# lucadellalib/audiocodecs

Hardware: AMD Instinct MI355X
Metric: encode+decode audio-sec/s, EnCodec-24k 8cb (higher is better)
Workload: dtype f32 (GEMM-shaped kernels and LSTM products: operands as two scaled fp16 planes, 3 partial products, fp32 accumulate -- split16.h)

## Files before the change

### audiocodecs_amd/csrc/ac_api.hip

```cpp
#include "core.h"
#include "tap_route.h"

extern "C" {

int ac_version(void) { return 400; }

int ac_create(const ac_config* cfg, ac_handle** out) {
    if (!cfg || !out) return AC_EINVAL;
    *out = nullptr;
    if (cfg->struct_size != (int32_t)sizeof(ac_config)) return AC_EINVAL;
    if (cfg->num_ratios < 1 || cfg->num_ratios > AC_MAX_RATIOS || cfg->num_filters < 1 || cfg->hidden_size < 16 ||
        cfg->hidden_size % 16 || cfg->compress < 1 || cfg->num_lstm_layers < 1 || cfg->num_lstm_layers > 2 || cfg->codebook_size % 32 ||
        cfg->codebook_size < 16 || cfg->num_quantizers < 1 || cfg->kernel_size < 1 || cfg->kernel_size > 8 ||
        cfg->last_kernel_size < 1 || cfg->last_kernel_size > 8 || cfg->residual_kernel_size < 1 || cfg->residual_kernel_size > 8)
        return AC_EINVAL;
    int ndev = 0;
    if (hipGetDeviceCount(&ndev) != hipSuccess || ndev <= cfg->device || cfg->device < 0) return AC_ENODEV;
    ac_handle* h = new (std::nothrow) ac_handle();
    if (!h) return AC_ENOMEM;
    h->cfg = *cfg;
    h->hop = 1;
    for (int i = 0; i < cfg->num_ratios; ++i) h->hop *= cfg->upsampling_ratios[i];
    h->D = cfg->num_filters << cfg->num_ratios;
    *out = h;
// ... 9 lines not shown
static std::string wavtok_key(const std::string& name) {
    static const std::string pre = "feature_extractor.encodec.encoder.model.";
    if (name.compare(0, pre.size(), pre) != 0) return name;
    std::string k = "encoder.layers." + name.substr(pre.size());
    const size_t cc = k.find(".conv.conv.");
    if (cc != std::string::npos) k = k.substr(0, cc) + ".conv." + k.substr(cc + 11);
    auto ends = [&](const char* sfx) { const size_t n = std::strlen(sfx); return k.size() >= n && k.compare(k.size() - n, n, sfx) == 0; };
    if (ends(".weight_g")) k = k.substr(0, k.size() - 9) + ".parametrizations.weight.original0";
    else if (ends(".weight_v")) k = k.substr(0, k.size() - 9) + ".parametrizations.weight.original1";
    return k;
}

int ac_load_weights(ac_handle* h, const char* name, const void* host_ptr, size_t bytes) {
    if (!h || !name || !host_ptr) return h ? fail(h, AC_EINVAL, "null argument") : AC_EINVAL;
    if (h->finalized) return fail(h, AC_ESTATE, "handle already finalized");
    if (bytes % 4) return fail(h, AC_EINVAL, "tensor '%s': byte size %zu is not a multiple of 4", name, bytes);
    const float* f = static_cast<const float*>(host_ptr);
    h->host[h->arch == ARCH_WAVTOK ? wavtok_key(name) : std::string(name)].assign(f, f + bytes / 4);
    return AC_OK;
}



static void latch_dev_switches(ac_handle* h) {
    auto num = [](const char* name, int dflt) { const char* v = std::getenv(name); return v && *v ? std::atoi(v) : dflt; };
    const char* e = std::getenv("AC_TAP_EPI");
    h->dev.tap_epi_staged = e && std::strcmp(e, "staged") == 0;
    h->dev.tap_dil = num("AC_TAP_DIL", 1);
    h->dev.tap_stagger = num("AC_TAP_STAGGER", 0);
    h->dev.tap_pick = num("AC_TAP_PICK", -1);
    h->dev.tap8 = num("AC_TAP8", -1);
    h->dev.tap8_form = num("AC_TAP8_FORM", 0);
    h->dev.tap8_spread = num("AC_TAP8_SPREAD", 1);
#ifdef AC_DEVELOPER
    h->dev.rb6_dbg = num("AC_RB6_DBG", 0);
    h->dev.lstm_dbg = num("AC_LSTM_DBG", 0);
#endif
    h->dev.rb_stream = num("AC_RB_STREAM", 1);
    h->dev.chain_stream = num("AC_CHAIN_STREAM", 1);
    h->dev.rb128_stream = num("AC_RB128_STREAM", 1);
    h->dev.front_seg = std::max(0, num("AC_FRONT_SEG", 0));
    h->dev.tail_seg = std::max(0, num("AC_TAIL_SEG", 0));
    h->dev.front_ldspad = std::max(0, num("AC_FRONT_LDSPAD", 0));
    h->dev.lstm_fuse_in = num("AC_LSTM_FUSE_IN", 1);
    const char* r = std::getenv("AC_RVQ");
    h->dev.rvq_exact = r && std::strcmp(r, "fp32") == 0;
    h->dev.prof_detail = num("AC_PROF_DETAIL", 0);
    h->dev.head_seq = num("AC_HEAD_SEQ", 0);
    h->dev.attn_exact = num("AC_ATTN_EXACT", 0);
    h->dev.dac_unit = num("AC_DAC_UNIT", 1);
    h->dev.mimi_tail = num("AC_MIMI_TAIL", 1);
    h->dev.mstream_skinny = num("AC_MSTREAM_SKINNY", -1);
}

int ac_debug_set(ac_handle* h, const char* key, int value) {
    if (!h || !key) return AC_EINVAL;
    struct { const char* k; int* v; } tab[] = {
        {"tap_epi_staged", &h->dev.tap_epi_staged}, {"tap_dil", &h->dev.tap_dil}, {"tap_stagger", &h->dev.tap_stagger}, {"tap_pick", &h->dev.tap_pick}, {"tap8", &h->dev.tap8}, {"tap8_form", &h->dev.tap8_form}, {"tap8_spread", &h->dev.tap8_spread},
        {"rb6_dbg", &h->dev.rb6_dbg}, {"rb_stream", &h->dev.rb_stream}, {"chain_stream", &h->dev.chain_stream}, {"rb128_stream", &h->dev.rb128_stream}, {"front_seg", &h->dev.front_seg}, {"tail_seg", &h->dev.tail_seg}, {"front_ldspad", &h->dev.front_ldspad},
        {"lstm_dbg", &h->dev.lstm_dbg}, {"lstm_fuse_in", &h->dev.lstm_fuse_in}, {"rvq_exact", &h->dev.rvq_exact}, {"prof_detail", &h->dev.prof_detail}, {"head_seq", &h->dev.head_seq}, {"attn_exact", &h->dev.attn_exact}, {"dac_unit", &h->dev.dac_unit}, {"mimi_tail", &h->dev.mimi_tail},
        {"mstream_skinny", &h->dev.mstream_skinny},
    };
#ifndef AC_DEVELOPER
    if (std::strcmp(key, "rb6_dbg") == 0 || std::strcmp(key, "lstm_dbg") == 0)
        return fail(h, AC_EINVAL, "ac_debug_set('%s'): a developer-build switch (timing modes with wrong results / fault injection); this is the product library", key);
#endif
    if (!h->finalized) return fail(h, AC_ESTATE, "ac_debug_set('%s'): the switches are latched by ac_finalize; set them afterwards", key);
    for (auto& t : tab)
        if (std::strcmp(t.k, key) == 0) {
            const bool nonneg = t.v == &h->dev.front_seg || t.v == &h->dev.tail_seg || t.v == &h->dev.front_ldspad || t.v == &h->dev.tap_stagger;
            if (nonneg && value < 0) return fail(h, AC_EINVAL, "ac_debug_set('%s', %d): the value must be >= 0", key, value);
            if (t.v == &h->dev.front_ldspad && value > 16384) return fail(h, AC_EINVAL, "ac_debug_set('front_ldspad', %d): at most 16384 bytes", value);
            if (t.v == &h->dev.tap8_form && (value < 0 || value > 5)) return fail(h, AC_EINVAL, "ac_debug_set('tap8_form', %d): 0 (cost model) .. 5", value);
            *t.v = value;
            return AC_OK;
        }
    return fail(h, AC_EINVAL, "ac_debug_set: unknown switch '%s'", key);
}

int ac_set_precision(ac_handle* h, int precision) {
    if (!h) return AC_EINVAL;
    if (h->finalized) return fail(h, AC_ESTATE, "ac_set_precision must precede ac_finalize (weights are packed for one arithmetic)");
    if (precision != AC_PRECISION_FP32 && precision != AC_PRECISION_FP32_EXACT) return fail(h, AC_EINVAL, "unknown precision %d", precision);
    h->precision = precision;
    return AC_OK;
}

int ac_finalize(ac_handle* h) {
    if (!h) return AC_EINVAL;
    if (h->finalized) return fail(h, AC_ESTATE, "handle already finalized");
    {
// ... 552 lines not shown
```

### audiocodecs_amd/csrc/core.h

```cpp
#pragma once
#include <hip/hip_runtime.h>

#include <algorithm>
#include <cmath>
#include <cstdarg>
#include <cstdio>
#include <cstdlib>
#include <cstring>
#include <map>
#include <string>
#include <vector>

#include "../../include/audiocodecs_amd.h"
#include "lstm_consts.h"
#include "rvq_types.h"
#include "split16.h"
#include "tap_gemm.h"

using namespace ac;

namespace ac {
constexpr int THIN_MAXK = 8;
struct RbFused6Params;
}
// ... 113 lines not shown
    int arch = ARCH_ENCODEC;
    ac_config cfg{};
    ac_mimi_config mcfg{};
    MimiPlan mimi;
    ac_dac_config dcfg{};
    DacPlan dac;
    ac_wavtok_config wcfg{};
    WavtokPlan wt;
    std::string err;
    std::map<std::string, std::vector<float>> host;
    bool finalized = false;
    float* blob = nullptr;
    size_t blob_floats = 0;
    int hop = 1, D = 0;
    PackedGemm enc_stem, enc_final;
    std::vector<ResBlockPlan> enc_rb;
    std::vector<PackedGemm> enc_down;
    LstmPlan enc_lstm, dec_lstm;
    PackedGemm dec_first, dec_head;
    std::vector<PackedGemm> dec_up;
    std::vector<ResBlockPlan> dec_rb;
    size_t cb_plain = 0, cb_packed = 0, cb_ee = 0;
    size_t cb16 = 0, cb16_inv = 0;
    struct ChainBounds { float sb0 = 0.f, sb1 = 0.f, fb0 = 0.f, fb1h = 0.f, fb1x = 0.f; bool ok = false; } enc_front, dec_tail;
    struct StreamImgs { size_t stem_f = 0, stem_inv = 0, down_f = 0, down_inv = 0, up_f = 0, up_inv = 0, head_f = 0, head_inv = 0; bool enc_ok = false, dec_ok = false; } simg;
    struct DevSwitches {
        int tap_epi_staged = 0;
        int tap_dil = 1;
        int tap_stagger = 0;
        int tap_pick = -1;
        int tap8 = -1;
        int tap8_form = 0;
        int tap8_spread = 1;
        int rb6_dbg = 0;
        int rb_stream = 1;
        int rb128_stream = 1;
        int chain_stream = 1;
        int front_seg = 0, tail_seg = 0;
        int front_ldspad = 0;
        int lstm_dbg = 0;
        int lstm_fuse_in = 1;
        int rvq_exact = 0;
        int prof_detail = 0;
        int attn_exact = 0;
        int dac_unit = 1;
        int mimi_tail = 1;
        int head_seq = 0;
        int mstream_skinny = -1;
    } dev;
    bool fuse_chains = true;
    float* dbg = nullptr;
    size_t dbg_cap = 0, dbg_used = 0;
    std::vector<const void*> lds_opted;
    std::map<size_t, size_t> w6_of;
    std::map<size_t, size_t> t6_of;
    std::map<size_t, size_t> t6inv_of;
    bool noncausal = false;
    bool has_enc = true, has_dec = true;
    bool gemm_fp32 = false;
    std::map<size_t, size_t> winv_of;
    std::map<const void*, int> mimi_streams;
    std::map<const void*, int> mimi_dstreams;
    struct EStreamReg { int B; bool fresh; };
    std::map<const void*, EStreamReg> encodec_streams, encodec_dstreams;
    unsigned* amax_buf = nullptr;
    int amax_B = 0, amax_next = 0;
// ... 744 lines not shown
```

### audiocodecs_amd/csrc/core.hip

```cpp
#include "core.h"
#include "split16_kernels.h"
#include "lstm.h"
#include "lstm_persist.h"
#include "lstm_persist16.h"
#include "rvq.h"
#include "rvq16.h"
#include "tap_gemm4.h"
#include "tap_gemm6.h"
#include "tap_gemm8.h"
#include "tap_route.h"
#include "thin.h"
#include "rb_fused.h"
#include "rb_fused6.h"
#include "thin_conv6.h"
#include "rb_fused6_128.h"
#include "enc_front.h"
#include "dec_tail.h"

namespace acimpl {


int fail(ac_handle* h, int code, const char* fmt, ...) {
    char buf[1024];
    va_list ap;
// ... 176 lines not shown
static int launch_tap6(ac_handle* h, hipStream_t st, TapGemmParams& p, const __bf16* w6, const char* name, double flops, double bytes) {
    using Cfg = Tap6Cfg<WGM, WGN, WMT, WN, HALO>;
    p.mtiles = cdiv(p.M, Cfg::BM);
    p.ntiles = p.N / Cfg::BN;
    const long long blocks = (long long)p.B * p.mtiles * p.ntiles;
    if (int rc = ensure_lds(h, reinterpret_cast<const void*>(tap_gemm6_kernel<WGM, WGN, WMT, WN, 2, HALO>), Cfg::lds_for(2))) return rc;
    ProfScope ps(h, st, name, flops, bytes);
    hipLaunchKernelGGL((tap_gemm6_kernel<WGM, WGN, WMT, WN, 2, HALO>), dim3((unsigned)blocks), dim3(Cfg::NT), Cfg::lds_for(2), st, p, w6);
    return AC_OK;
}

static int launch_tap6_family(ac_handle* h, hipStream_t st, TapGemmParams& p, const TapRoute& r, const __bf16* w6, const char* name, double flops, double bytes) {
    if (r.family == TapFamily::tap6_dil) {
        switch (r.key()) {
        case tap_key(1, 4, 4, 2): return launch_tap6<1, 4, 4, 2, T6_DIL_HALO>(h, st, p, w6, name, flops, bytes);
        case tap_key(1, 4, 4, 1): return launch_tap6<1, 4, 4, 1, T6_DIL_HALO>(h, st, p, w6, name, flops, bytes);
        case tap_key(2, 2, 2, 3): return launch_tap6<2, 2, 2, 3, T6_DIL_HALO>(h, st, p, w6, name, flops, bytes);
        case tap_key(4, 1, 1, 3): return launch_tap6<4, 1, 1, 3, T6_DIL_HALO>(h, st, p, w6, name, flops, bytes);
        }
    } else {
        switch (r.key()) {
        case tap_key(1, 4, 4, 2): return launch_tap6<1, 4, 4, 2, 7>(h, st, p, w6, name, flops, bytes);
        case tap_key(1, 8, 4, 1): return launch_tap6<1, 8, 4, 1, 7>(h, st, p, w6, name, flops, bytes);
        case tap_key(1, 4, 4, 1): return launch_tap6<1, 4, 4, 1, 7>(h, st, p, w6, name, flops, bytes);
        case tap_key(2, 2, 2, 3): return launch_tap6<2, 2, 2, 3, 7>(h, st, p, w6, name, flops, bytes);
        case tap_key(4, 1, 1, 3): return launch_tap6<4, 1, 1, 3, 7>(h, st, p, w6, name, flops, bytes);
        case tap_key(2, 2, 2, 1): return launch_tap6<2, 2, 2, 1, 7>(h, st, p, w6, name, flops, bytes);
        }
    }
    return fail(h, AC_EINVAL, "run_tap: no instantiation of %s", r.name);
}

template <int WGM, int WGN, int WMT, int WN, bool RM, bool J1, bool SP>
static int launch_tap8(ac_handle* h, hipStream_t st, TapGemmParams& p, const __bf16* w6, const char* name, double flops, double bytes) {
    using Cfg = Tap8Cfg<WGM, WGN, WMT, WN>;
    p.mtiles = cdiv(p.M, Cfg::BM);
    p.ntiles = p.N / Cfg::BN;
    const long long blocks = (long long)p.B * p.mtiles * p.ntiles;
    ProfScope ps(h, st, name, flops, bytes);
    if (int rc = ensure_lds(h, reinterpret_cast<const void*>(tap_gemm8_kernel<WGM, WGN, WMT, WN, RM, J1, SP>), Cfg::lds_bytes)) return rc;
    hipLaunchKernelGGL((tap_gemm8_kernel<WGM, WGN, WMT, WN, RM, J1, SP>), dim3((unsigned)blocks), dim3(Cfg::NT), Cfg::lds_bytes, st, p, w6);
    return AC_OK;
}

static int launch_tap8_family(ac_handle* h, hipStream_t st, TapGemmParams& p, const TapRoute& r, const __bf16* w6, const char* name, double flops, double bytes) {
    constexpr int RJ = TK_RM | TK_J1, J = TK_J1, S = TK_SPREAD;
    switch (r.key()) {
    case tap_key(2, 4, 4, 2, RJ): return launch_tap8<2, 4, 4, 2, true, true, false>(h, st, p, w6, name, flops, bytes);
    case tap_key(2, 4, 4, 2, RJ | S): return launch_tap8<2, 4, 4, 2, true, true, true>(h, st, p, w6, name, flops, bytes);
    case tap_key(2, 4, 4, 2, J): return launch_tap8<2, 4, 4, 2, false, true, false>(h, st, p, w6, name, flops, bytes);
    case tap_key(2, 4, 4, 2, J | S): return launch_tap8<2, 4, 4, 2, false, true, true>(h, st, p, w6, name, flops, bytes);
    case tap_key(2, 4, 4, 2): return launch_tap8<2, 4, 4, 2, false, false, false>(h, st, p, w6, name, flops, bytes);
    case tap_key(2, 4, 4, 2, S): return launch_tap8<2, 4, 4, 2, false, false, true>(h, st, p, w6, name, flops, bytes);
    case tap_key(2, 4, 2, 2, RJ): return launch_tap8<2, 4, 2, 2, true, true, false>(h, st, p, w6, name, flops, bytes);
    case tap_key(2, 4, 2, 2, RJ | S): return launch_tap8<2, 4, 2, 2, true, true, true>(h, st, p, w6, name, flops, bytes);
    case tap_key(2, 4, 2, 2, J): return launch_tap8<2, 4, 2, 2, false, true, false>(h, st, p, w6, name, flops, bytes);
    case tap_key(2, 4, 2, 2, J | S): return launch_tap8<2, 4, 2, 2, false, true, true>(h, st, p, w6, name, flops, bytes);
    case tap_key(2, 4, 2, 2): return launch_tap8<2, 4, 2, 2, false, false, false>(h, st, p, w6, name, flops, bytes);
    case tap_key(2, 4, 2, 2, S): return launch_tap8<2, 4, 2, 2, false, false, true>(h, st, p, w6, name, flops, bytes);
    case tap_key(4, 2, 2, 2, RJ): return launch_tap8<4, 2, 2, 2, true, true, false>(h, st, p, w6, name, flops, bytes);
    case tap_key(4, 2, 2, 2, RJ | S): return launch_tap8<4, 2, 2, 2, true, true, true>(h, st, p, w6, name, flops, bytes);
    case tap_key(4, 2, 2, 2, J): return launch_tap8<4, 2, 2, 2, false, true, false>(h, st, p, w6, name, flops, bytes);
    case tap_key(4, 2, 2, 2, J | S): return launch_tap8<4, 2, 2, 2, false, true, true>(h, st, p, w6, name, flops, bytes);
    case tap_key(4, 2, 2, 2): return launch_tap8<4, 2, 2, 2, false, false, false>(h, st, p, w6, name, flops, bytes);
    case tap_key(4, 2, 2, 2, S): return launch_tap8<4, 2, 2, 2, false, false, true>(h, st, p, w6, name, flops, bytes);
    }
    return fail(h, AC_EINVAL, "run_tap: no instantiation of %s", r.name);
}


TapSeg make_seg(const Act& x, int s, int J, int pad , int extra, int kofs, const float* rel_len, int left, int right) {
    TapSeg g{};
    g.x = x.p;
    g.amax = x.amax;
    g.amax_n = x.amax_n;
    g.bs = x.bs;
    g.ts = x.ts;
    g.rel_len = rel_len;
    g.L = x.L;
    g.cin = x.C;
    g.cin_shift = -1;
    for (int sh = 0; sh < 30; ++sh)
        if ((1 << sh) == x.C) g.cin_shift = sh;
    g.s = s;
    g.J = J;
    const int pad_left = left < 0 ? (J - 1) * s : left;
    const int max_pad = std::max(pad_left, right + extra);
    g.Lp = (pad == PAD_REFLECT && x.L <= max_pad) ? max_pad + 1 : x.L;
    g.lim = pad != PAD_ZERO ? x.L + right + extra : x.L;
    g.reflect = pad;
    g.elu = 0;
    g.kofs = kofs;
    g.pad = pad_left;
    g.dil = 1;
    return g;
}


// ... 1158 lines not shown
```

### audiocodecs_amd/csrc/tap_gemm8.h

```cpp
#pragma once
#include "tap_gemm6.h"

namespace ac {

template <int WGM, int WGN, int WMT, int WN>
struct Tap8Cfg {
    using C6 = Tap6Cfg<WGM, WGN, WMT, WN, 7>;
    static_assert(WGM * WGN == 8, "8 waves");
    static constexpr int BM = C6::BM, BN = C6::BN, NT = C6::NT, A_ROWS = C6::A_ROWS, A_SLOTS = C6::A_SLOTS, PLANE = C6::PLANE;
    static constexpr int NTILES = BN / 32;
    static constexpr int B_PIECES = 2 * NTILES * 2;
    static constexpr int B_SLOT = B_PIECES * 512;
    static constexpr int PPW = B_PIECES / 8;
    static_assert(B_PIECES % 8 == 0, "fragments divide over the 8 waves");
    static constexpr size_t a_bytes = (size_t)2 * 2 * PLANE * 2;
    static constexpr size_t b_bytes = (size_t)2 * B_SLOT * 2;
    static_assert(a_bytes % 16 == 0, "ring base alignment");
    static constexpr size_t main_bytes = a_bytes + b_bytes;
    static constexpr size_t lds_bytes = main_bytes > C6::epi_bytes ? main_bytes : C6::epi_bytes;
    static_assert(lds_bytes <= 160 * 1024, "one workgroup per CU: slabs + weight ring (or the staged epilogue's tile) within 160 KB of LDS");
};

__device__ __forceinline__ void t8_glds16(const void* gsrc, unsigned lds_dst) {
#ifdef T8_ABL_NODMA
    return;
#endif
    unsigned keep;
    asm volatile("s_mov_b32 %0, m0\n\ts_mov_b32 m0, %2\n\ts_nop 0\n\tglobal_load_lds_dwordx4 %1, off\n\ts_mov_b32 m0, %0"
                 : "=&s"(keep) : "v"(gsrc), "s"(lds_dst) : "memory");
}
template <int N>
__device__ __forceinline__ void t8_wait() {
    asm volatile("s_waitcnt vmcnt(%0)" ::"n"(N) : "memory");
}

template <int WGM, int WGN, int WMT, int WN, bool RM, bool J1, bool SPREAD = true>
__global__ __launch_bounds__(512, 1) void tap_gemm8_kernel(const TapGemmParams p, const __bf16* __restrict__ wp) {
    using Cfg = Tap8Cfg<WGM, WGN, WMT, WN>;
    constexpr int BM = Cfg::BM, BN = Cfg::BN, NT = Cfg::NT, A_SLOTS = Cfg::A_SLOTS, PLANE = Cfg::PLANE, NTILES = Cfg::NTILES;
    constexpr int HALO = 7;
    unsigned long long clk_t0 = 0, clk_r0 = 0;
    if (p.clk) { clk_t0 = __builtin_amdgcn_s_memtime(); clk_r0 = __builtin_amdgcn_s_memrealtime(); }
    extern __shared__ __attribute__((aligned(16))) float smem[];
    __bf16* As0 = reinterpret_cast<__bf16*>(smem);
    __bf16* Bs0 = reinterpret_cast<__bf16*>(reinterpret_cast<char*>(smem) + Cfg::a_bytes);
    const unsigned bs_lds = (unsigned)(size_t)Bs0;

    const int tid = threadIdx.x, lane = tid & 63;
    const int wave = __builtin_amdgcn_readfirstlane(tid >> 6);
    const int wm = wave / WGN, wn = wave % WGN;
    const int i32 = lane & 31, kh = lane >> 5;

    int id;
    {
        const int total = gridDim.x, q = total >> 3, r = total & 7, xcd = blockIdx.x & 7, pos = blockIdx.x >> 3;
        id = (xcd < r ? xcd * (q + 1) : r * (q + 1) + (xcd - r) * q) + pos;
    }
    const int nt = id % p.ntiles; id /= p.ntiles;
    const int mt = id % p.mtiles;
    const int b = id / p.mtiles;
    const int m0 = mt * BM, n0 = nt * BN;
#ifdef T6_TRACE
    const bool t6_ph = p.clk && mt == p.mtiles / 2 && nt == 0 && b == p.B / 2 && tid == 64;
    const bool t8_on = p.clk && mt == p.mtiles / 2 && nt == 0 && b == p.B / 2 && lane == 0;
    int t8_stage = 0;
    if (t6_ph) p.clk[4] = clk_t0;
#define T8_STAMP(k) do { if (t8_on && t8_stage < 16) p.clk[16 + (wave * 16 + t8_stage) * 8 + (k)] = __builtin_amdgcn_s_memtime(); } while (0)
#define T8_USTAMP(u) do { if (t8_on && (t8_stage == 2 || t8_stage == 3) && (u) < 8) p.clk[16 + (wave * 16 + 8 + (u)) * 8 + 3 + t8_stage] = __builtin_amdgcn_s_memtime(); } while (0)
    T6_PHASE(1);
#else
    const bool t6_ph = false;
#define T8_STAMP(k) do { } while (0)
#define T8_USTAMP(u) do { } while (0)
#endif

    const TapSeg& sg = p.seg[0];
    const unsigned am_early = RM ? 0u : *amax_at(sg.amax, b);
    const int seg_J = sg.J, seg_Cw = sg.s * sg.cin, seg_kofs = sg.kofs, rowstep = sg.dil;
    const int NC = seg_Cw / KC;
    const long long lo_t = (long long)m0 * sg.s - sg.pad;
    const long long hi_t = (long long)(m0 + BM - 1 + (sg.J - 1) * sg.dil) * sg.s + (sg.s - 1) - sg.pad;
    const bool inside = lo_t >= 0 && hi_t < sg.L;
    const bool seg_interior = inside || sg.s == 1;
    const int tsf = sg.s == 1 ? (int)sg.ts : sg.cin;
    const __amdgpu_buffer_rsrc_t a_rs = __builtin_amdgcn_make_buffer_rsrc((void*)(sg.x + (long long)b * sg.bs), 0,
                                                                             (int)(((long long)(sg.L - 1) * sg.ts + sg.cin) * 4), 0x00020000);
    const int R = BM + (sg.J - 1) * sg.dil;
    int a_boff[A_SLOTS];
    const int a_lds0 = (tid / (KC / 4)) * T6_PITCH + 4 * (tid % (KC / 4));
    const bool last_slot_ok = (tid + (A_SLOTS - 1) * NT) / (KC / 4) < Cfg::A_ROWS;
    unsigned a_zero = 0;
#pragma unroll
    for (int i = 0; i < A_SLOTS; ++i) {
        const int e = tid + i * NT;
        const int row = e / (KC / 4), q = e % (KC / 4);
        long long t = (long long)(m0 + (row < R ? row : 0)) * sg.s - sg.pad;
        if (!inside) {
            if (sg.s == 1) {
                const long long jj = row < R ? src_index(sg, (int)t) : 0;
                if (jj < 0) a_zero |= 1u << i;
                t = jj < 0 ? 0 : jj;
            } else {
                t = 0;
            }
        }
        a_boff[i] = (int)((t * tsf + 4 * q) * 4);
    }
    __builtin_amdgcn_sched_barrier(0);
    float a_scale = 1.f, a_inv = 1.f;
    float a_rsc[RM ? A_SLOTS : 1];
    constexpr bool rowmode = RM;
    if (!RM) {
        unsigned am = am_early;
        asm volatile("" : "+v"(am));
        const int se = s16_exponent(am);
        a_scale = s16_pow2(se);
        a_inv = s16_pow2(-se);
        a_rsc[0] = a_scale;
    } else {
#pragma unroll
        for (int i = 0; i < A_SLOTS; ++i) {
            const int m = m0 + (tid + i * NT) / (KC / 4);
            a_rsc[RM ? i : 0] = s16_pow2(s16_exponent(sg.amax[m < p.M ? m : p.M - 1]));
        }
    }

    f32x16 acc[WMT][WN];
#pragma unroll
    for (int a = 0; a < WMT; ++a)
#pragma unroll
        for (int c = 0; c < WN; ++c)
#pragma unroll
            for (int r = 0; r < 16; ++r) acc[a][c][r] = 0.f;

    constexpr int A_OOB = 0x7fff0000;
    const __amdgpu_buffer_rsrc_t a_rs_null = __builtin_amdgcn_make_buffer_rsrc((void*)(sg.x + (long long)b * sg.bs), 0, 0, 0x00020000);
    auto load_a = [&](int c, bool live, f32x4 (&ra)[A_SLOTS]) {
#ifdef T8_ABL_NOALOAD
        live = false;
#endif
        const int c_ = c * KC;
        if (seg_interior || !live) {
            const int soff = __builtin_amdgcn_readfirstlane(live ? c_ * 4 : 0);
            const __amdgpu_buffer_rsrc_t rs = live ? a_rs : a_rs_null;
#pragma unroll
            for (int i = 0; i < A_SLOTS; ++i) ra[i] = bufload16(rs, a_boff[i], soff);
        } else {
            int voff[A_SLOTS];
#pragma unroll
            for (int i = 0; i < A_SLOTS; ++i) {
                const int e = tid + i * NT;
                const int row = e / (KC / 4), q = e % (KC / 4);
                const int cc = c_ + 4 * q;
                const int tp = sg.cin_shift >= 0 ? (cc >> sg.cin_shift) : (cc / sg.cin);
                const long long jj = row < R ? src_index(sg, (m0 + row) * sg.s + tp - sg.pad) : -1;
                voff[i] = jj < 0 ? A_OOB : (int)((jj * sg.ts + (cc - tp * sg.cin)) * 4);
            }
#pragma unroll
            for (int i = 0; i < A_SLOTS; ++i) ra[i] = bufload16(a_rs, voff[i], 0);
        }
    };
    auto load_slot = [&](int c, bool live, f32x4 (&ra)[A_SLOTS], int i) {
#ifdef T8_ABL_NOALOAD
        live = false;
#endif
        const int c_ = c * KC;
        if (seg_interior || !live) {
            const int soff = __builtin_amdgcn_readfirstlane(live ? c_ * 4 : 0);
            const __amdgpu_buffer_rsrc_t rs = live ? a_rs : a_rs_null;
            ra[i] = bufload16(rs, a_boff[i], soff);
        } else {
            const int e = tid + i * NT;
            const int row = e / (KC / 4), q = e % (KC / 4);
            const int cc = c_ + 4 * q;
            const int tp = sg.cin_shift >= 0 ? (cc >> sg.cin_shift) : (cc / sg.cin);
            const long long jj = row < R ? src_index(sg, (m0 + row) * sg.s + tp - sg.pad) : -1;
            ra[i] = bufload16(a_rs, jj < 0 ? A_OOB : (int)((jj * sg.ts + (cc - tp * sg.cin)) * 4), 0);
        }
    };
    auto store_slot = [&](const f32x4 (&ra)[A_SLOTS], __bf16* dst, int i) {
        if (i + 1 == A_SLOTS) asm volatile("" ::"v"(ra[i]));
#ifdef T8_ABL_NOSTORE
        return;
#endif
        if (i + 1 < A_SLOTS || last_slot_ok) {
            const f32x4 v = (a_zero & (1u << i)) ? f32x4{0.f, 0.f, 0.f, 0.f} : ra[i];
            split16_store4s(v, a_rsc[RM ? i : 0], dst, PLANE, a_lds0 + i * (NT / (KC / 4)) * T6_PITCH);
        }
    };
    auto store_a = [&](const f32x4 (&ra)[A_SLOTS], __bf16* dst) {
#pragma unroll
        for (int i = 0; i < A_SLOTS; ++i) store_slot(ra, dst, i);
    };
    const int ksteps = p.Ktot >> 4;
    const __bf16* wtile = wp + (long long)(n0 >> 5) * ksteps * 1024 + lane * 8;
    auto issue_b = [&](int c, int j, int slot) {
        const int k0 = (seg_kofs + j * seg_Cw + c * KC) >> 4;
#pragma unroll
        for (int i = 0; i < Cfg::PPW; ++i) {
            const int f = wave * Cfg::PPW + i;
            const int ks = f / (2 * NTILES), t = (f / 2) % NTILES, pl = f % 2;
            t8_glds16(wtile + ((long long)t * ksteps + k0 + ks) * 1024 + pl * 512, bs_lds + (unsigned)((slot * Cfg::B_PIECES + f) * 1024));
        }
    };

    auto issue_piece = [&](int c, int j, int slot, int i) {
        const int k0 = (seg_kofs + j * seg_Cw + c * KC) >> 4;
        const int f = wave * Cfg::PPW + i;
        const int ks = f / (2 * NTILES), t = (f / 2) % NTILES, pl = f % 2;
        t8_glds16(wtile + ((long long)t * ksteps + k0 + ks) * 1024 + pl * 512, bs_lds + (unsigned)((slot * Cfg::B_PIECES + f) * 1024));
    };

    const int a_frag = (wm * WMT * 32 + i32) * T6_PITCH + 8 * kh;
    auto compute = [&](int abuf, int jr, int slot, auto&& hook) {
        const __bf16* Ac = As0 + abuf * 2 * PLANE + a_frag + jr * T6_PITCH;
        const __bf16* Bc = Bs0 + slot * Cfg::B_SLOT + lane * 8;
        f16x8 bf[2][2][WN], af[2][2];
        auto read_b = [&](int ks, f16x8 (&dst)[2][WN]) {
#pragma unroll
            for (int c = 0; c < WN; ++c)
#pragma unroll
                for (int pl = 0; pl < 2; ++pl) dst[pl][c] = *reinterpret_cast<const f16x8*>(Bc + ((ks * NTILES + wn * WN + c) * 2 + pl) * 512);
        };
        auto read_a = [&](int ks, int a, f16x8 (&dst)[2]) {
#pragma unroll
            for (int pl = 0; pl < 2; ++pl) dst[pl] = *reinterpret_cast<const f16x8*>(Ac + pl * PLANE + a * 32 * T6_PITCH + ks * 16);
        };
        read_b(0, bf[0]);
// ... 20 lines not shown
        }
    };
    auto no_hook = [](int) {};
    constexpr int UNITS = 2 * WMT;
    constexpr int SPU = (A_SLOTS + UNITS - 1) / UNITS, SU0 = UNITS - (A_SLOTS + SPU - 1) / SPU;
    auto store_hook = [&](const f32x4 (&ra)[A_SLOTS], __bf16* dst, bool st, int u) {
        if (u >= SU0 && st) {
#pragma unroll
            for (int k = 0; k < SPU; ++k)
                if ((u - SU0) * SPU + k < A_SLOTS) store_slot(ra, dst, (u - SU0) * SPU + k);
        }
    };

    auto tasks = [&](int u, bool has_next, int nc, int nj, int nslot, bool issue, int creq, f32x4 (&ra_req)[A_SLOTS], bool store, const f32x4 (&ra_st)[A_SLOTS], __bf16* dst,
                     auto issue_tag, auto store_tag) {
        constexpr bool ISSUE = decltype(issue_tag)::value, STORE = decltype(store_tag)::value;
        constexpr int NTASK = Cfg::PPW + (ISSUE ? A_SLOTS : 0) + (STORE ? A_SLOTS : 0);
        const int lo = u * NTASK / UNITS, hi = (u + 1) * NTASK / UNITS;
#pragma unroll
        for (int t = 0; t < NTASK; ++t) {
            if (t < lo || t >= hi) continue;
            if (t < Cfg::PPW) {
                if (has_next) issue_piece(nc, nj, nslot, t);
            } else if (ISSUE && t < Cfg::PPW + A_SLOTS) {
                load_slot(creq, issue, ra_req, t - Cfg::PPW);
            } else {
                if (store) store_slot(ra_st, dst, t - Cfg::PPW - (ISSUE ? A_SLOTS : 0));
            }
        }
    };

    using T = std::true_type;
    using F = std::false_type;
#pragma unroll
    for (int i = 0; i < (RM ? A_SLOTS : 1); ++i) asm volatile("" ::"v"(a_rsc[i]));
#ifdef T6_TRACE
    T6_PHASE(2);
#endif
    if constexpr (J1) {
        f32x4 raA[A_SLOTS], raB[A_SLOTS];
        issue_b(0, 0, 0);
        load_a(0, true, raA);
        load_a(1, NC > 1, raB);
        store_a(raA, As0);
        t8_wait<A_SLOTS>();
        lds_barrier();
#ifdef T6_TRACE
        T6_PHASE(6);
#endif
        auto stage = [&](int c, f32x4 (&ra_next)[A_SLOTS], f32x4 (&ra_free)[A_SLOTS]) {
            T8_STAMP(0);
            const bool st = c + 1 < NC;
            __bf16* dst = As0 + ((c + 1) & 1) * 2 * PLANE;
            if constexpr (SPREAD) {
                T8_STAMP(1);
                compute(c & 1, 0, c & 1, [&](int u) { tasks(u, c + 1 < NC, c + 1, 0, (c + 1) & 1, c + 2 < NC, c + 2, ra_free, st, ra_next, dst, T{}, T{}); });
            } else {
                if (c + 1 < NC) issue_b(c + 1, 0, (c + 1) & 1);
                load_a(c + 2, c + 2 < NC, ra_free);
                __builtin_amdgcn_sched_barrier(0);
                T8_STAMP(1);
                compute(c & 1, 0, c & 1, [&](int u) { store_hook(ra_next, dst, st, u); });
            }
            __builtin_amdgcn_sched_barrier(0);
            T8_STAMP(2);
            t8_wait<A_SLOTS>();
            T8_STAMP(3);
            lds_barrier();
            T8_STAMP(4);
#ifdef T6_TRACE
            ++t8_stage;
#endif
        };
        for (int c = 0; c < NC; c += 2) {
            stage(c, raB, raA);
            if (c + 1 < NC) stage(c + 1, raA, raB);
        }
    } else {
        f32x4 ra[A_SLOTS];
        issue_b(0, 0, 0);
        load_a(0, true, ra);
        store_a(ra, As0);
        load_a(1, NC > 1, ra);
        t8_wait<A_SLOTS>();
        lds_barrier();
#ifdef T6_TRACE
        T6_PHASE(6);
#endif
        auto stage = [&](int c, int j, auto store_tag, auto issue_tag) {
            constexpr bool STORE = decltype(store_tag)::value, ISSUE = decltype(issue_tag)::value;
            const int s = c * seg_J + j;
            int nc = c, nj = j + 1;
            if (nj == seg_J) { nj = 0; nc = c + 1; }
            T8_STAMP(0);
            if constexpr (SPREAD) {
                T8_STAMP(1);
                const bool st = c + 1 < NC;
                __bf16* dst = As0 + ((c + 1) & 1) * 2 * PLANE;
                compute(c & 1, j * rowstep, s & 1, [&](int u) { tasks(u, nc < NC, nc, nj, (s + 1) & 1, c + 2 < NC, c + 2, ra, st, ra, dst, issue_tag, store_tag); });
            } else {
            if (nc < NC) issue_b(nc, nj, (s + 1) & 1);
            if (ISSUE) load_a(c + 2, c + 2 < NC, ra);
            __builtin_amdgcn_sched_barrier(0);
            T8_STAMP(1);
            if constexpr (STORE) {
                const bool st = c + 1 < NC;
                __bf16* dst = As0 + ((c + 1) & 1) * 2 * PLANE;
                compute(c & 1, j * rowstep, s & 1, [&](int u) { store_hook(ra, dst, st, u); });
            } else {
                compute(c & 1, j * rowstep, s & 1, no_hook);
            }
            }
            __builtin_amdgcn_sched_barrier(0);
            T8_STAMP(2);
            if (ISSUE) t8_wait<A_SLOTS>(); else t8_wait<0>();
            T8_STAMP(3);
            lds_barrier();
            T8_STAMP(4);
#ifdef T6_TRACE
            ++t8_stage;
#endif
        };
        for (int c = 0; c < NC; ++c) {
            stage(c, 0, T{}, F{});
            for (int j = 1; j < seg_J - 1; ++j) stage(c, j, F{}, F{});
            stage(c, seg_J - 1, F{}, T{});
        }
    }

    tap6_epilogue<WGM, WGN, WMT, WN, HALO>(p, acc, smem, b, m0, n0, a_inv, rowmode, clk_t0, clk_r0, t6_ph);
#undef T8_STAMP
#undef T8_USTAMP
}

}
```

### audiocodecs_amd/csrc/tap_route.h

```cpp
#pragma once
#include "core.h"

namespace acimpl {

struct TapRouteInputs {
    bool w6 = false;
    bool winv = false;
    bool want_rowmode = false;
    bool want_rows = false;
    bool gemm_fp32 = false;
};

enum class TapFamily { scalar, vec, tap4, tap6, tap6_dil, tap8 };

enum { TK_RM = 1, TK_J1 = 2, TK_SPREAD = 4 };
constexpr int tap_key(int wgm, int wgn, int wm, int wn, int flags = 0) { return flags << 16 | wgm << 12 | wgn << 8 | wm << 4 | wn; }

struct TapRoute {
    int reject_taps = 0;
    TapFamily family = TapFamily::scalar;
    int wgm = 0, wgn = 0, wm = 0, wn = 0;
    int form8 = 0;
    bool rm = false, j1 = false, spread = false;
    bool rowmode = false;
    bool rows_out = false;
    bool epi_direct = false;
    bool dil_slab = false;
    char name[48] = "";
    int key() const { return tap_key(wgm, wgn, wm, wn, (rm ? TK_RM : 0) | (j1 ? TK_J1 : 0) | (spread ? TK_SPREAD : 0)); }
};

inline void tap_route_set(TapRoute& r, TapFamily f, int wgm, int wgn, int wm, int wn) {
    r.family = f;
    r.wgm = wgm;
    r.wgn = wgn;
    r.wm = wm;
    r.wn = wn;
    const char* fmt = f == TapFamily::scalar   ? "tap_gemm_kernel<%d, %d, %d, %d, false>"
                      : f == TapFamily::vec    ? "tap_gemm_kernel<%d, %d, %d, %d, true>"
                      : f == TapFamily::tap4   ? "tap_gemm4_kernel<%d, %d, %d, %d>"
                      : f == TapFamily::tap6   ? "tap_gemm6_kernel<%d, %d, %d, %d, 2>"
                      : f == TapFamily::tap6_dil ? "tap_gemm6_kernel<%d, %d, %d, %d, 2, dil>"
                                                 : "tap_gemm8_kernel<%d, %d, %d, %d, 2>";
    std::snprintf(r.name, sizeof r.name, fmt, wgm, wgn, wm, wn);
}

inline TapRoute route_tap(const TapGemmParams& p, const TapRouteInputs& in, const ac_handle::DevSwitches& dev) {
    TapRoute r;
    bool vec = (p.Ktot % 4 == 0) && aligned16(p.w);
    bool fast = vec && (p.N % 4 == 0) && (p.y_rs % 4 == 0) && (p.y_bs % 4 == 0) && (!p.y || aligned16(p.y)) &&
                (!p.y_elu || aligned16(p.y_elu)) && (long long)p.N * p.Ktot * 4 < (1LL << 31);
    for (int i = 0; i < p.nseg; ++i) {
        const TapSeg& s = p.seg[i];
        vec = vec && (s.cin % 4 == 0) && (s.ts % 4 == 0) && (s.bs % 4 == 0) && (s.kofs % 4 == 0) && aligned16(s.x);
        fast = fast && ((s.s * s.cin) % KC == 0) && (s.ts == s.cin || s.s == 1) && !s.rel_len && !s.elu &&
               ((long long)(s.L - 1) * s.ts + s.cin) * 4 < (1LL << 31);
// ... 28 lines not shown
    }
    const bool dil_env = dev.tap_dil != 0;
    r.dil_slab = dil_env && !r.rowmode && p.nseg == 1 && p.seg[0].dil != 1    && p.seg[0].s == 1 && (p.seg[0].J - 1) * p.seg[0].dil <= T6_DIL_HALO;
    const TapSeg& s0 = p.seg[0];
    const bool can8 = in.winv && p.nseg == 1 && (s0.J - 1) * s0.dil <= 7 && !(s0.dil != 1 && s0.s != 1) && p.N % 128 == 0 && (s0.s * s0.cin) % 32 == 0 &&
                      (!r.epi_direct || p.N % 128 == 0);
    const int want8 = dev.tap8;
    if (can8 && want8 != 0) {
        auto fill8 = [&](int bm, int bn) {
            const double w = (double)p.B * cdiv(p.M, bm) * (p.N / bn) / 256.0;
            return w / std::ceil(w) * ((double)p.M / ((double)cdiv(p.M, bm) * bm));
        };
        const double sc1 = p.N % 256 == 0 ? 1.00 * fill8(256, 256) : 0.0;
        const double sc3 = p.N % 256 == 0 ? 0.90 * fill8(128, 256) : 0.0;
        int form = sc1 >= sc3 ? 1 : 3;
        bool model = (form == 1 ? sc1 : sc3) >= 0.80;
        if (p.N % 256 != 0) {
            form = 2;
            model = kk >= 3072 && fill8(256, 128) >= 0.70;
        }
        if ((double)p.B * cdiv(p.M, 128) * (p.N / 128) <= 64.0) {
            form = p.N % 256 == 0 ? 3 : 2;
            model = true;
        }
        if (dev.tap8_form >= 1 && dev.tap8_form <= 3 && (dev.tap8_form == 2 || p.N % 256 == 0)) form = dev.tap8_form;
        if (want8 >= 1 || model) {
            r.form8 = form;
            if (form == 1) tap_route_set(r, TapFamily::tap8, 2, 4, 4, 2);
            else if (form == 3) tap_route_set(r, TapFamily::tap8, 2, 4, 2, 2);
            else tap_route_set(r, TapFamily::tap8, 4, 2, 2, 2);
            r.j1 = s0.J == 1;
            r.rm = r.j1 && r.rowmode;
            r.spread = dev.tap8_spread == 2 || (dev.tap8_spread == 1 && r.wgm * r.wm * 32 == 128);
            return r;
        }
    }
    int pick = 0;
    if (p.N % 256 == 0) {
        const double wg256 = (double)p.B * cdiv(p.M, 128) * (p.N / 256);
        auto fill = [](double wgs, double slots) { const double w = wgs / slots; return w / std::ceil(w); };
        const double s128 = in.winv ? 1.06 * fill(2.0 * wg256, 768.0) : 1.00 * fill(2.0 * wg256, 512.0);
        const double s256 = 1.10 * fill(wg256, 512.0);
        const double s8 = (kk >= 2048 ? (in.winv ? 1.00 : 1.12) : (in.winv ? 0.85 : 0.95)) * fill(wg256, 256.0);
        pick = s256 >= s128 && s256 >= s8 ? 1 : (s8 > s128 ? 2 : 0);
        if (dev.tap_pick >= 0 && dev.tap_pick <= 2) pick = dev.tap_pick;
    }
    auto tap6 = [&](int wgm, int wgn, int wmt, int wn) {
        const bool dil = in.winv && r.dil_slab && (wn >= 2 || (wgm == 1 && wgn == 4 && kk >= 2048));
        tap_route_set(r, dil ? TapFamily::tap6_dil : TapFamily::tap6, wgm, wgn, wmt, wn);
    };
    if (pick == 1) tap6(1, 4, 4, 2);
    else if (pick == 2) tap6(1, 8, 4, 1);
    else if (p.N % 128 == 0) tap6(1, 4, 4, 1);
    else if (p.N % 192 == 0) tap6(2, 2, 2, 3);
    else if (p.N % 96 == 0) tap6(4, 1, 1, 3);
    else tap6(2, 2, 2, 1);
    return r;
}

}
```

Measured before the change: 41970.

## Make tap8 GEMM kernel persistent over tiles with next-tile prefetch under epilogue

For J1 tap8 configurations with small per-wave tiles, the launch now uses at most one workgroup per CU. Each workgroup walks a strided list of tiles within its XCD partition. Per-tile setup (batch resource descriptors, A offsets, scales, weight pointer) moves into a lambda. When the direct epilogue is used, the next tile's first A and B loads are issued before the current epilogue so they overlap. This cuts launch and workgroup startup cost and hides prologue latency, at the risk of losing occupancy or parallelism when the tile count is only slightly above the CU count.

```diff
diff --git a/audiocodecs_amd/csrc/ac_api.hip b/audiocodecs_amd/csrc/ac_api.hip
--- a/audiocodecs_amd/csrc/ac_api.hip
+++ b/audiocodecs_amd/csrc/ac_api.hip
@@ -65,6 +65,7 @@
     h->dev.tap8 = num("AC_TAP8", -1);
     h->dev.tap8_form = num("AC_TAP8_FORM", 0);
     h->dev.tap8_spread = num("AC_TAP8_SPREAD", 1);
+    h->dev.tap8_persist = num("AC_TAP8_PERSIST", 1);
 #ifdef AC_DEVELOPER
     h->dev.rb6_dbg = num("AC_RB6_DBG", 0);
     h->dev.lstm_dbg = num("AC_LSTM_DBG", 0);
@@ -89,7 +90,7 @@
 int ac_debug_set(ac_handle* h, const char* key, int value) {
     if (!h || !key) return AC_EINVAL;
     struct { const char* k; int* v; } tab[] = {
-        {"tap_epi_staged", &h->dev.tap_epi_staged}, {"tap_dil", &h->dev.tap_dil}, {"tap_stagger", &h->dev.tap_stagger}, {"tap_pick", &h->dev.tap_pick}, {"tap8", &h->dev.tap8}, {"tap8_form", &h->dev.tap8_form}, {"tap8_spread", &h->dev.tap8_spread},
+        {"tap_epi_staged", &h->dev.tap_epi_staged}, {"tap_dil", &h->dev.tap_dil}, {"tap_stagger", &h->dev.tap_stagger}, {"tap_pick", &h->dev.tap_pick}, {"tap8", &h->dev.tap8}, {"tap8_form", &h->dev.tap8_form}, {"tap8_spread", &h->dev.tap8_spread}, {"tap8_persist", &h->dev.tap8_persist},
         {"rb6_dbg", &h->dev.rb6_dbg}, {"rb_stream", &h->dev.rb_stream}, {"chain_stream", &h->dev.chain_stream}, {"rb128_stream", &h->dev.rb128_stream}, {"front_seg", &h->dev.front_seg}, {"tail_seg", &h->dev.tail_seg}, {"front_ldspad", &h->dev.front_ldspad},
         {"lstm_dbg", &h->dev.lstm_dbg}, {"lstm_fuse_in", &h->dev.lstm_fuse_in}, {"rvq_exact", &h->dev.rvq_exact}, {"prof_detail", &h->dev.prof_detail}, {"head_seq", &h->dev.head_seq}, {"attn_exact", &h->dev.attn_exact}, {"dac_unit", &h->dev.dac_unit}, {"mimi_tail", &h->dev.mimi_tail},
         {"mstream_skinny", &h->dev.mstream_skinny},
diff --git a/audiocodecs_amd/csrc/core.h b/audiocodecs_amd/csrc/core.h
--- a/audiocodecs_amd/csrc/core.h
+++ b/audiocodecs_amd/csrc/core.h
@@ -169,6 +169,7 @@
         int tap8 = -1;
         int tap8_form = 0;
         int tap8_spread = 1;
+        int tap8_persist = 1;
         int rb6_dbg = 0;
         int rb_stream = 1;
         int rb128_stream = 1;
diff --git a/audiocodecs_amd/csrc/core.hip b/audiocodecs_amd/csrc/core.hip
--- a/audiocodecs_amd/csrc/core.hip
+++ b/audiocodecs_amd/csrc/core.hip
@@ -232,11 +232,13 @@
 }
 
 template <int WGM, int WGN, int WMT, int WN, bool RM, bool J1, bool SP>
-static int launch_tap8(ac_handle* h, hipStream_t st, TapGemmParams& p, const __bf16* w6, const char* name, double flops, double bytes) {
+static int launch_tap8(ac_handle* h, hipStream_t st, TapGemmParams& p, const __bf16* w6, bool persist, const char* name, double flops, double bytes) {
     using Cfg = Tap8Cfg<WGM, WGN, WMT, WN>;
     p.mtiles = cdiv(p.M, Cfg::BM);
     p.ntiles = p.N / Cfg::BN;
-    const long long blocks = (long long)p.B * p.mtiles * p.ntiles;
+    const long long tiles = (long long)p.B * p.mtiles * p.ntiles;
+    if (tiles <= 0 || tiles > 0x7fffffffLL) return fail(h, AC_EINVAL, "run_tap: %lld tiles", tiles);
+    const long long blocks = persist && Cfg::PERSIST && J1 ? std::min(tiles, (long long)std::max(h->num_cus, 8)) : tiles;
     ProfScope ps(h, st, name, flops, bytes);
     if (int rc = ensure_lds(h, reinterpret_cast<const void*>(tap_gemm8_kernel<WGM, WGN, WMT, WN, RM, J1, SP>), Cfg::lds_bytes)) return rc;
     hipLaunchKernelGGL((tap_gemm8_kernel<WGM, WGN, WMT, WN, RM, J1, SP>), dim3((unsigned)blocks), dim3(Cfg::NT), Cfg::lds_bytes, st, p, w6);
@@ -246,24 +248,24 @@
 static int launch_tap8_family(ac_handle* h, hipStream_t st, TapGemmParams& p, const TapRoute& r, const __bf16* w6, const char* name, double flops, double bytes) {
     constexpr int RJ = TK_RM | TK_J1, J = TK_J1, S = TK_SPREAD;
     switch (r.key()) {
-    case tap_key(2, 4, 4, 2, RJ): return launch_tap8<2, 4, 4, 2, true, true, false>(h, st, p, w6, name, flops, bytes);
-    case tap_key(2, 4, 4, 2, RJ | S): return launch_tap8<2, 4, 4, 2, true, true, true>(h, st, p, w6, name, flops, bytes);
-    case tap_key(2, 4, 4, 2, J): return launch_tap8<2, 4, 4, 2, false, true, false>(h, st, p, w6, name, flops, bytes);
-    case tap_key(2, 4, 4, 2, J | S): return launch_tap8<2, 4, 4, 2, false, true, true>(h, st, p, w6, name, flops, bytes);
-    case tap_key(2, 4, 4, 2): return launch_tap8<2, 4, 4, 2, false, false, false>(h, st, p, w6, name, flops, bytes);
-    case tap_key(2, 4, 4, 2, S): return launch_tap8<2, 4, 4, 2, false, false, true>(h, st, p, w6, name, flops, bytes);
-    case tap_key(2, 4, 2, 2, RJ): return launch_tap8<2, 4, 2, 2, true, true, false>(h, st, p, w6, name, flops, bytes);
-    case tap_key(2, 4, 2, 2, RJ | S): return launch_tap8<2, 4, 2, 2, true, true, true>(h, st, p, w6, name, flops, bytes);
-    case tap_key(2, 4, 2, 2, J): return launch_tap8<2, 4, 2, 2, false, true, false>(h, st, p, w6, name, flops, bytes);
-    case tap_key(2, 4, 2, 2, J | S): return launch_tap8<2, 4, 2, 2, false, true, true>(h, st, p, w6, name, flops, bytes);
-    case tap_key(2, 4, 2, 2): return launch_tap8<2, 4, 2, 2, false, false, false>(h, st, p, w6, name, flops, bytes);
-    case tap_key(2, 4, 2, 2, S): return launch_tap8<2, 4, 2, 2, false, false, true>(h, st, p, w6, name, flops, bytes);
-    case tap_key(4, 2, 2, 2, RJ): return launch_tap8<4, 2, 2, 2, true, true, false>(h, st, p, w6, name, flops, bytes);
-    case tap_key(4, 2, 2, 2, RJ | S): return launch_tap8<4, 2, 2, 2, true, true, true>(h, st, p, w6, name, flops, bytes);
-    case tap_key(4, 2, 2, 2, J): return launch_tap8<4, 2, 2, 2, false, true, false>(h, st, p, w6, name, flops, bytes);
-    case tap_key(4, 2, 2, 2, J | S): return launch_tap8<4, 2, 2, 2, false, true, true>(h, st, p, w6, name, flops, bytes);
-    case tap_key(4, 2, 2, 2): return launch_tap8<4, 2, 2, 2, false, false, false>(h, st, p, w6, name, flops, bytes);
-    case tap_key(4, 2, 2, 2, S): return launch_tap8<4, 2, 2, 2, false, false, true>(h, st, p, w6, name, flops, bytes);
+    case tap_key(2, 4, 4, 2, RJ): return launch_tap8<2, 4, 4, 2, true, true, false>(h, st, p, w6, r.persist, name, flops, bytes);
+    case tap_key(2, 4, 4, 2, RJ | S): return launch_tap8<2, 4, 4, 2, true, true, true>(h, st, p, w6, r.persist, name, flops, bytes);
+    case tap_key(2, 4, 4, 2, J): return launch_tap8<2, 4, 4, 2, false, true, false>(h, st, p, w6, r.persist, name, flops, bytes);
+    case tap_key(2, 4, 4, 2, J | S): return launch_tap8<2, 4, 4, 2, false, true, true>(h, st, p, w6, r.persist, name, flops, bytes);
+    case tap_key(2, 4, 4, 2): return launch_tap8<2, 4, 4, 2, false, false, false>(h, st, p, w6, r.persist, name, flops, bytes);
+    case tap_key(2, 4, 4, 2, S): return launch_tap8<2, 4, 4, 2, false, false, true>(h, st, p, w6, r.persist, name, flops, bytes);
+    case tap_key(2, 4, 2, 2, RJ): return launch_tap8<2, 4, 2, 2, true, true, false>(h, st, p, w6, r.persist, name, flops, bytes);
+    case tap_key(2, 4, 2, 2, RJ | S): return launch_tap8<2, 4, 2, 2, true, true, true>(h, st, p, w6, r.persist, name, flops, bytes);
+    case tap_key(2, 4, 2, 2, J): return launch_tap8<2, 4, 2, 2, false, true, false>(h, st, p, w6, r.persist, name, flops, bytes);
+    case tap_key(2, 4, 2, 2, J | S): return launch_tap8<2, 4, 2, 2, false, true, true>(h, st, p, w6, r.persist, name, flops, bytes);
+    case tap_key(2, 4, 2, 2): return launch_tap8<2, 4, 2, 2, false, false, false>(h, st, p, w6, r.persist, name, flops, bytes);
+    case tap_key(2, 4, 2, 2, S): return launch_tap8<2, 4, 2, 2, false, false, true>(h, st, p, w6, r.persist, name, flops, bytes);
+    case tap_key(4, 2, 2, 2, RJ): return launch_tap8<4, 2, 2, 2, true, true, false>(h, st, p, w6, r.persist, name, flops, bytes);
+    case tap_key(4, 2, 2, 2, RJ | S): return launch_tap8<4, 2, 2, 2, true, true, true>(h, st, p, w6, r.persist, name, flops, bytes);
+    case tap_key(4, 2, 2, 2, J): return launch_tap8<4, 2, 2, 2, false, true, false>(h, st, p, w6, r.persist, name, flops, bytes);
+    case tap_key(4, 2, 2, 2, J | S): return launch_tap8<4, 2, 2, 2, false, true, true>(h, st, p, w6, r.persist, name, flops, bytes);
+    case tap_key(4, 2, 2, 2): return launch_tap8<4, 2, 2, 2, false, false, false>(h, st, p, w6, r.persist, name, flops, bytes);
+    case tap_key(4, 2, 2, 2, S): return launch_tap8<4, 2, 2, 2, false, false, true>(h, st, p, w6, r.persist, name, flops, bytes);
     }
     return fail(h, AC_EINVAL, "run_tap: no instantiation of %s", r.name);
 }
diff --git a/audiocodecs_amd/csrc/tap_gemm8.h b/audiocodecs_amd/csrc/tap_gemm8.h
--- a/audiocodecs_amd/csrc/tap_gemm8.h
+++ b/audiocodecs_amd/csrc/tap_gemm8.h
@@ -18,6 +18,7 @@
     static_assert(a_bytes % 16 == 0, "ring base alignment");
     static constexpr size_t main_bytes = a_bytes + b_bytes;
     static constexpr size_t lds_bytes = main_bytes > C6::epi_bytes ? main_bytes : C6::epi_bytes;
+    static constexpr bool PERSIST = WMT * WN * 16 <= 64;
     static_assert(lds_bytes <= 160 * 1024, "one workgroup per CU: slabs + weight ring (or the staged epilogue's tile) within 160 KB of LDS");
 };
 
@@ -39,8 +40,8 @@
     using Cfg = Tap8Cfg<WGM, WGN, WMT, WN>;
     constexpr int BM = Cfg::BM, BN = Cfg::BN, NT = Cfg::NT, A_SLOTS = Cfg::A_SLOTS, PLANE = Cfg::PLANE, NTILES = Cfg::NTILES;
     constexpr int HALO = 7;
+    constexpr bool WALK = Cfg::PERSIST && J1;
     unsigned long long clk_t0 = 0, clk_r0 = 0;
-    if (p.clk) { clk_t0 = __builtin_amdgcn_s_memtime(); clk_r0 = __builtin_amdgcn_s_memrealtime(); }
     extern __shared__ __attribute__((aligned(16))) float smem[];
     __bf16* As0 = reinterpret_cast<__bf16*>(smem);
     __bf16* Bs0 = reinterpret_cast<__bf16*>(reinterpret_cast<char*>(smem) + Cfg::a_bytes);
@@ -51,23 +52,20 @@
     const int wm = wave / WGN, wn = wave % WGN;
     const int i32 = lane & 31, kh = lane >> 5;
 
-    int id;
+    int tile, tile_end, tile_step;
     {
-        const int total = gridDim.x, q = total >> 3, r = total & 7, xcd = blockIdx.x & 7, pos = blockIdx.x >> 3;
-        id = (xcd < r ? xcd * (q + 1) : r * (q + 1) + (xcd - r) * q) + pos;
+        const int tiles = p.B * p.mtiles * p.ntiles, q = tiles >> 3, r = tiles & 7, G = gridDim.x, xcd = blockIdx.x & 7, pos = blockIdx.x >> 3;
+        const int first = xcd < r ? xcd * (q + 1) : r * (q + 1) + (xcd - r) * q;
+        tile_end = first + q + (xcd < r ? 1 : 0);
+        tile_step = (G >> 3) + (xcd < (G & 7) ? 1 : 0);
+        tile = first + pos;
     }
-    const int nt = id % p.ntiles; id /= p.ntiles;
-    const int mt = id % p.mtiles;
-    const int b = id / p.mtiles;
-    const int m0 = mt * BM, n0 = nt * BN;
-#ifdef T6_TRACE
-    const bool t6_ph = p.clk && mt == p.mtiles / 2 && nt == 0 && b == p.B / 2 && tid == 64;
-    const bool t8_on = p.clk && mt == p.mtiles / 2 && nt == 0 && b == p.B / 2 && lane == 0;
+    if (tile >= tile_end) return;
+#ifdef T6_TRACE
+    bool t6_ph = false, t8_on = false;
     int t8_stage = 0;
-    if (t6_ph) p.clk[4] = clk_t0;
 #define T8_STAMP(k) do { if (t8_on && t8_stage < 16) p.clk[16 + (wave * 16 + t8_stage) * 8 + (k)] = __builtin_amdgcn_s_memtime(); } while (0)
 #define T8_USTAMP(u) do { if (t8_on && (t8_stage == 2 || t8_stage == 3) && (u) < 8) p.clk[16 + (wave * 16 + 8 + (u)) * 8 + 3 + t8_stage] = __builtin_amdgcn_s_memtime(); } while (0)
-    T6_PHASE(1);
 #else
     const bool t6_ph = false;
 #define T8_STAMP(k) do { } while (0)
@@ -75,66 +73,87 @@
 #endif
 
     const TapSeg& sg = p.seg[0];
-    const unsigned am_early = RM ? 0u : *amax_at(sg.amax, b);
     const int seg_J = sg.J, seg_Cw = sg.s * sg.cin, seg_kofs = sg.kofs, rowstep = sg.dil;
     const int NC = seg_Cw / KC;
-    const long long lo_t = (long long)m0 * sg.s - sg.pad;
-    const long long hi_t = (long long)(m0 + BM - 1 + (sg.J - 1) * sg.dil) * sg.s + (sg.s - 1) - sg.pad;
-    const bool inside = lo_t >= 0 && hi_t < sg.L;
-    const bool seg_interior = inside || sg.s == 1;
     const int tsf = sg.s == 1 ? (int)sg.ts : sg.cin;
-    const __amdgpu_buffer_rsrc_t a_rs = __builtin_amdgcn_make_buffer_rsrc((void*)(sg.x + (long long)b * sg.bs), 0,
-                                                                             (int)(((long long)(sg.L - 1) * sg.ts + sg.cin) * 4), 0x00020000);
+    const int a_records = (int)(((long long)(sg.L - 1) * sg.ts + sg.cin) * 4);
     const int R = BM + (sg.J - 1) * sg.dil;
-    int a_boff[A_SLOTS];
     const int a_lds0 = (tid / (KC / 4)) * T6_PITCH + 4 * (tid % (KC / 4));
     const bool last_slot_ok = (tid + (A_SLOTS - 1) * NT) / (KC / 4) < Cfg::A_ROWS;
+    const int ksteps = p.Ktot >> 4;
+    constexpr bool rowmode = RM;
+
+    int b = -1, m0 = 0, n0 = 0;
+    bool inside = false, seg_interior = false;
+    __amdgpu_buffer_rsrc_t a_rs, a_rs_null;
+    int a_boff[A_SLOTS];
     unsigned a_zero = 0;
-#pragma unroll
-    for (int i = 0; i < A_SLOTS; ++i) {
-        const int e = tid + i * NT;
-        const int row = e / (KC / 4), q = e % (KC / 4);
-        long long t = (long long)(m0 + (row < R ? row : 0)) * sg.s - sg.pad;
-        if (!inside) {
-            if (sg.s == 1) {
-                const long long jj = row < R ? src_index(sg, (int)t) : 0;
-                if (jj < 0) a_zero |= 1u << i;
-                t = jj < 0 ? 0 : jj;
-            } else {
-                t = 0;
-            }
-        }
-        a_boff[i] = (int)((t * tsf + 4 * q) * 4);
-    }
-    __builtin_amdgcn_sched_barrier(0);
+    unsigned am_word = 0;
     float a_scale = 1.f, a_inv = 1.f;
     float a_rsc[RM ? A_SLOTS : 1];
-    constexpr bool rowmode = RM;
-    if (!RM) {
-        unsigned am = am_early;
-        asm volatile("" : "+v"(am));
-        const int se = s16_exponent(am);
-        a_scale = s16_pow2(se);
-        a_inv = s16_pow2(-se);
-        a_rsc[0] = a_scale;
-    } else {
+    const __bf16* wtile = wp;
+    auto setup_tile = [&](int id) {
+        int tid_ = tid;
+        asm volatile("" : "+v"(tid_));
+        const int nt = id % p.ntiles; id /= p.ntiles;
+        const int mt = id % p.mtiles;
+        const int nb = id / p.mtiles;
+        m0 = mt * BM, n0 = nt * BN;
+#ifdef T6_TRACE
+        t6_ph = p.clk && mt == p.mtiles / 2 && nt == 0 && nb == p.B / 2 && tid == 64;
+        t8_on = p.clk && mt == p.mtiles / 2 && nt == 0 && nb == p.B / 2 && lane == 0;
+        t8_stage = 0;
+#endif
+        if (nb != b) {
+            if (!RM) am_word = *amax_at(sg.amax, nb);
+            b = nb;
+            a_rs = __builtin_amdgcn_make_buffer_rsrc((void*)(sg.x + (long long)b * sg.bs), 0, a_records, 0x00020000);
+            a_rs_null = __builtin_amdgcn_make_buffer_rsrc((void*)(sg.x + (long long)b * sg.bs), 0, 0, 0x00020000);
+        }
+        const long long lo_t = (long long)m0 * sg.s - sg.pad;
+        const long long hi_t = (long long)(m0 + BM - 1 + (sg.J - 1) * sg.dil) * sg.s + (sg.s - 1) - sg.pad;
+        inside = lo_t >= 0 && hi_t < sg.L;
+        seg_interior = inside || sg.s == 1;
+        a_zero = 0;
 #pragma unroll
         for (int i = 0; i < A_SLOTS; ++i) {
-            const int m = m0 + (tid + i * NT) / (KC / 4);
-            a_rsc[RM ? i : 0] = s16_pow2(s16_exponent(sg.amax[m < p.M ? m : p.M - 1]));
-        }
-    }
+            const int e = tid_ + i * NT;
+            const int row = e / (KC / 4), q = e % (KC / 4);
+            long long t = (long long)(m0 + (row < R ? row : 0)) * sg.s - sg.pad;
+            if (!inside) {
+                if (sg.s == 1) {
+                    const long long jj = row < R ? src_index(sg, (int)t) : 0;
+                    if (jj < 0) a_zero |= 1u << i;
+                    t = jj < 0 ? 0 : jj;
+                } else {
+                    t = 0;
+                }
+            }
+            a_boff[i] = (int)((t * tsf + 4 * q) * 4);
+        }
+        __builtin_amdgcn_sched_barrier(0);
+        if (!RM) {
+            unsigned am = am_word;
+            asm volatile("" : "+v"(am));
+            const int se = s16_exponent(am);
+            a_scale = s16_pow2(se);
+            a_inv = s16_pow2(-se);
+            a_rsc[0] = a_scale;
+        } else {
+#pragma unroll
+            for (int i = 0; i < A_SLOTS; ++i) {
+                const int m = m0 + (tid_ + i * NT) / (KC / 4);
+                a_rsc[RM ? i : 0] = s16_pow2(s16_exponent(sg.amax[m < p.M ? m : p.M - 1]));
+            }
+        }
+        wtile = wp + (long long)(n0 >> 5) * ksteps * 1024 + (tid_ & 63) * 8;
+#pragma unroll
+        for (int i = 0; i < (RM ? A_SLOTS : 1); ++i) asm volatile("" ::"v"(a_rsc[i]));
+    };
 
     f32x16 acc[WMT][WN];
-#pragma unroll
-    for (int a = 0; a < WMT; ++a)
-#pragma unroll
-        for (int c = 0; c < WN; ++c)
-#pragma unroll
-            for (int r = 0; r < 16; ++r) acc[a][c][r] = 0.f;
 
     constexpr int A_OOB = 0x7fff0000;
-    const __amdgpu_buffer_rsrc_t a_rs_null = __builtin_amdgcn_make_buffer_rsrc((void*)(sg.x + (long long)b * sg.bs), 0, 0, 0x00020000);
     auto load_a = [&](int c, bool live, f32x4 (&ra)[A_SLOTS]) {
 #ifdef T8_ABL_NOALOAD
         live = false;
@@ -192,8 +211,6 @@
 #pragma unroll
         for (int i = 0; i < A_SLOTS; ++i) store_slot(ra, dst, i);
     };
-    const int ksteps = p.Ktot >> 4;
-    const __bf16* wtile = wp + (long long)(n0 >> 5) * ksteps * 1024 + lane * 8;
     auto issue_b = [&](int c, int j, int slot) {
         const int k0 = (seg_kofs + j * seg_Cw + c * KC) >> 4;
 #pragma unroll
@@ -280,15 +297,26 @@
 
     using T = std::true_type;
     using F = std::false_type;
-#pragma unroll
-    for (int i = 0; i < (RM ? A_SLOTS : 1); ++i) asm volatile("" ::"v"(a_rsc[i]));
-#ifdef T6_TRACE
-    T6_PHASE(2);
-#endif
-    if constexpr (J1) {
-        f32x4 raA[A_SLOTS], raB[A_SLOTS];
+    f32x4 raA[A_SLOTS], raB[J1 ? A_SLOTS : 1];
+    auto prefetch = [&]() {
         issue_b(0, 0, 0);
         load_a(0, true, raA);
+    };
+    setup_tile(tile);
+    prefetch();
+    for (;;) {
+    if (p.clk) { clk_t0 = __builtin_amdgcn_s_memtime(); clk_r0 = __builtin_amdgcn_s_memrealtime(); }
+#ifdef T6_TRACE
+    if (t6_ph) p.clk[4] = clk_t0;
+    T6_PHASE(2);
+#endif
+#pragma unroll
+    for (int a = 0; a < WMT; ++a)
+#pragma unroll
+        for (int c = 0; c < WN; ++c)
+#pragma unroll
+            for (int r = 0; r < 16; ++r) acc[a][c][r] = 0.f;
+    if constexpr (J1) {
         load_a(1, NC > 1, raB);
         store_a(raA, As0);
         t8_wait<A_SLOTS>();
@@ -325,9 +353,7 @@
             if (c + 1 < NC) stage(c + 1, raA, raB);
         }
     } else {
-        f32x4 ra[A_SLOTS];
-        issue_b(0, 0, 0);
-        load_a(0, true, ra);
+        f32x4 (&ra)[A_SLOTS] = raA;
         store_a(ra, As0);
         load_a(1, NC > 1, ra);
         t8_wait<A_SLOTS>();
@@ -376,7 +402,25 @@
         }
     }
 
-    tap6_epilogue<WGM, WGN, WMT, WN, HALO>(p, acc, smem, b, m0, n0, a_inv, rowmode, clk_t0, clk_r0, t6_ph);
+    const int e_b = b, e_m0 = m0, e_n0 = n0;
+    const float e_inv = a_inv;
+    const bool e_ph = t6_ph;
+    const int tile_next = tile + tile_step;
+    const bool has_next = WALK && tile_next < tile_end, direct = p.epi_direct != 0;
+    if (has_next && direct) {
+        setup_tile(tile_next);
+        prefetch();
+    }
+    tap6_epilogue<WGM, WGN, WMT, WN, HALO>(p, acc, smem, e_b, e_m0, e_n0, e_inv, rowmode, clk_t0, clk_r0, e_ph);
+    if (!has_next) break;
+    if (!direct) {
+        lds_barrier();
+        setup_tile(tile_next);
+        prefetch();
+    }
+    tile = tile_next;
+    }
+    if constexpr (WALK) __builtin_amdgcn_s_waitcnt(0x0F70);
 #undef T8_STAMP
 #undef T8_USTAMP
 }
diff --git a/audiocodecs_amd/csrc/tap_route.h b/audiocodecs_amd/csrc/tap_route.h
--- a/audiocodecs_amd/csrc/tap_route.h
+++ b/audiocodecs_amd/csrc/tap_route.h
@@ -22,6 +22,7 @@
     int wgm = 0, wgn = 0, wm = 0, wn = 0;
     int form8 = 0;
     bool rm = false, j1 = false, spread = false;
+    bool persist = false;
     bool rowmode = false;
     bool rows_out = false;
     bool epi_direct = false;
@@ -116,6 +117,7 @@
             r.j1 = s0.J == 1;
             r.rm = r.j1 && r.rowmode;
             r.spread = dev.tap8_spread == 2 || (dev.tap8_spread == 1 && r.wgm * r.wm * 32 == 128);
+            r.persist = dev.tap8_persist != 0;
             return r;
         }
     }
```

New measurement: 41860. About the same (-0.3%).
